# codeMonkey339/Congestion-control-with-BitTorren

Measured on AMD Instinct MI355X. Metric: GiB/s device-resident SHA-1 over 512KB chunks; % of HBM-read roofline, higher is better.
Workload: dtype u32; 1 GPU; 4096 x 524288 B chunks per GPU, device-resident (BASELINE config 2); chunks_per_gpu=4096, chunk_bytes=524288, kernel=split_u4_2prod, kernel_requested=auto, streams=1, parallelism=chunk-sharded x1, no collective

## Files before the change

### congestion-control-with-bittorren_amd/csrc/rt_device.hip

```cpp
#include <algorithm>
#include <atomic>
#include <cctype>
#include <cstdarg>
#include <cstdio>
#include <cstdlib>
#include <cstring>
#include <mutex>
#include <sched.h>
#include <string>
#include <vector>

#include "sha1_runtime_internal.h"

using namespace s1rt;

namespace {
std::atomic<uint64_t> g_launches[kLaunchCounters];

std::string sysfs_line(const char* path) {
    char buf[4096] = {0};
    if (FILE* f = fopen(path, "r")) {
        if (!fgets(buf, sizeof buf, f)) buf[0] = 0;
        fclose(f);
    }
// ... 69 lines not shown
    std::call_once(n.once, [&] {
        if (numa_off()) return;
        cpu_set_t allowed, mine;
        if (!s1host::process_cpus(&allowed)) return;
        constexpr int kMinNearCpus = 4;
        if (device_node_cpus(id, allowed, &mine) < kMinNearCpus || CPU_EQUAL(&mine, &allowed)) return;
        n.set = mine;
        n.ok = true;
    });
    return n.ok ? &n.set : nullptr;
}

const std::vector<cpu_set_t>& receive_domains(int id) {
    struct Dom {
        std::once_flag once;
        std::vector<cpu_set_t> dom;
    };
    static Dom doms[64];
    static const std::vector<cpu_set_t> none;
    if (id < 0 || id >= 64) return none;
    Dom& d = doms[id];
    std::call_once(d.once, [&] {
        cpu_set_t allowed, base;
        if (!s1host::process_cpus(&allowed)) return;
        if (numa_off() || device_node_cpus(id, allowed, &base) == 0) base = allowed;
        s1host::l3_domains(base, &d.dom, [](int cpu) {
            char path[128];
            snprintf(path, sizeof path, "/sys/devices/system/cpu/cpu%d/cache/index3/shared_cpu_list", cpu);
            return sysfs_line(path);
        });
    });
    return d.dom;
}

thread_local int t_dev = 0;

int fail(int code, const char* fmt, ...) {
    char buf[512];
    va_list ap;
    va_start(ap, fmt);
    vsnprintf(buf, sizeof buf, fmt, ap);
    va_end(ap);
    t_err = buf;
    return code;
}

std::string g_probe_err;
Device* g_dev = nullptr;

int device_count() {
    std::call_once(g_once, probe);
    return g_count;
}

int ensure_slots(Device& D, int n) {
    for (int i = 0; i < n && i < kMaxSlots; ++i) {
        Slot& s = D.slot[i];
        if (s.stream) continue;
        HIP_TRY(hipEventCreateWithFlags(&s.done, hipEventDisableTiming));
        HIP_TRY(hipEventCreateWithFlags(&s.copied, hipEventDisableTiming));
        HIP_TRY(hipStreamCreateWithFlags(&s.stream, hipStreamNonBlocking));
    }
    return SHA1CHUNK_OK;
}

int ensure_copy(Device& D) {
    if (!D.copy) HIP_TRY(hipStreamCreateWithFlags(&D.copy, hipStreamNonBlocking));
    return SHA1CHUNK_OK;
}

int get_device(Device** out) {
    if (device_count() <= 0) return fail(SHA1CHUNK_ENODEV, "%s", g_probe_err.c_str());
    if (t_dev < 0 || t_dev >= g_count) return fail(SHA1CHUNK_EINVAL, "bad device %d", t_dev);
    Device& D = g_dev[t_dev];
    HIP_TRY(hipSetDevice(D.id));
    if (!D.ready.load(std::memory_order_acquire)) {
        std::lock_guard<std::mutex> lk(D.mu);
        if (!D.ready.load(std::memory_order_relaxed)) {
            hipDeviceProp_t pr;
            HIP_TRY(hipGetDeviceProperties(&pr, D.id));
            D.cus = pr.multiProcessorCount;
            int rc = ensure_slots(D, 1);
            if (rc) return rc;
            D.ready.store(true, std::memory_order_release);
        }
    }
    *out = &D;
    return SHA1CHUNK_OK;
}

int copies_issued(Slot& s, hipStream_t cs) {
    if (cs == s.stream) return SHA1CHUNK_OK;
    HIP_TRY(hipEventRecord(s.copied, cs));
    HIP_TRY(hipStreamWaitEvent(s.stream, s.copied, 0));
    return SHA1CHUNK_OK;
}

int discard_in_flight(Device& D) {
    for (auto& s : D.slot) {
        if (!s.busy) continue;
        s.busy = false;
        HIP_TRY(hipEventSynchronize(s.done));
    }
    return SHA1CHUNK_OK;
}

int drain_cus_take(Device* D) {
    const int want = static_cast<int>(
        std::max<uint64_t>(1, std::min<uint64_t>({static_cast<uint64_t>(D->cus), 1024, env_u64("SHA1CHUNK_VQ_CUS", 64)})));
    const int budget = static_cast<int>(std::min<uint64_t>(
        static_cast<uint64_t>(D->cus), env_u64("SHA1CHUNK_VQ_CU_BUDGET", static_cast<uint64_t>(D->cus / 2))));
    std::lock_guard<std::mutex> lk(D->drain_mu);
    const int left = budget - D->drain_cus;
    const int take = std::min(want, left);
    if (take < std::min(want, 8)) return 0;
    D->drain_cus += take;
    return take;
}

void drain_cus_give(int dev, int cus) {
    if (dev < 0 || dev >= g_count) return;
    std::lock_guard<std::mutex> lk(g_dev[dev].drain_mu);
    g_dev[dev].drain_cus -= cus;
}

int drain_cus_held() {
    if (!g_dev || t_dev < 0 || t_dev >= g_count) return 0;
    std::lock_guard<std::mutex> lk(g_dev[t_dev].drain_mu);
    return g_dev[t_dev].drain_cus;
}
}

extern "C" {

int s1be_device_count(void) {
    const int n = device_count();
    if (n <= 0) fail(SHA1CHUNK_ENODEV, "%s", g_probe_err.c_str());
    return n;
}

int s1be_set_device(int device) {
    const int n = device_count();
    if (n <= 0) return fail(SHA1CHUNK_ENODEV, "%s", g_probe_err.c_str());
    if (device < 0 || device >= n) return fail(SHA1CHUNK_EINVAL, "device %d of %d", device, n);
    t_dev = device;
    return SHA1CHUNK_OK;
}

const char* s1be_last_error(void) { return t_err.c_str(); }

int s1be_device_pci_bus_id(int device, char* buf, size_t len) {
    const int n = device_count();
    if (n <= 0) return fail(SHA1CHUNK_ENODEV, "%s", g_probe_err.c_str());
    if (device < 0 || device >= n) return fail(SHA1CHUNK_EINVAL, "device %d of %d", device, n);
    if (len > static_cast<size_t>(INT32_MAX)) len = INT32_MAX;
    HIP_TRY(hipDeviceGetPCIBusId(buf, static_cast<int>(len), g_dev[device].id));
    return SHA1CHUNK_OK;
}

int s1be_receive_cpus(int device, unsigned slot, void* mask, size_t len, unsigned* domains) {
    const int n = device_count();
    if (n <= 0) return fail(SHA1CHUNK_ENODEV, "%s", g_probe_err.c_str());
    if (device < 0 || device >= n) return fail(SHA1CHUNK_EINVAL, "device %d of %d", device, n);
    const std::vector<cpu_set_t>& dom = receive_domains(g_dev[device].id);
    if (dom.empty()) return fail(SHA1CHUNK_EINVAL, "no CPU of this process's affinity mask found");
    const cpu_set_t& d = dom[slot % dom.size()];
// ... 18 lines not shown
```

### congestion-control-with-bittorren_amd/csrc/sha1_kernels.h

```cpp
#pragma once

#include <hip/hip_runtime.h>
#include <stdint.h>

struct BatchArgs {
    const uint8_t* base;
    const uint64_t* off;
    const uint32_t* len;
    uint32_t ulen;
    uint32_t n;
    const uint32_t* order;
    uint8_t* dig;
    const uint32_t* init_state;
    uint64_t prefix_bytes;
    uint32_t* out_state;
    const uint32_t* plan;
};

enum LaunchCounter {
    kLaunchLane, kLaunchFused, kLaunchSplit1, kLaunchSplit4, kLaunchSplit11Lane, kLaunchSplit11Shared,
    kLaunchQuad, kLaunchStudy, kLaunchMixed, kLaunchSort, kLaunchDrain, kLaunchCounters
};
void count_launch(LaunchCounter which);

hipError_t launch_lane(const BatchArgs& A, hipStream_t st);
hipError_t launch_fused(const BatchArgs& A, hipStream_t st);
constexpr int kSplitUnitQuad = 416;
bool split_unit_built(int unit_blocks);
hipError_t launch_split(const BatchArgs& A, int unit_blocks, hipStream_t st);
bool split_unit_study_built(int unit_blocks);
hipError_t launch_split_study(const BatchArgs& A, int unit_blocks, hipStream_t st);
uint32_t mixed_grid(uint32_t groups, int cus, uint32_t* hcap);
constexpr uint32_t kBigExact = 4096;
struct BigFix {
    const uint32_t* cnt;
    uint32_t tiles;
    const uint32_t* len;
    const uint32_t* id;
    uint32_t* order;
    uint32_t* sorted_len;
};
hipError_t launch_mixed(const BatchArgs& A, const uint32_t* sorted_len, const BigFix* big, uint32_t* plan, int cus,
                        const int* forced, hipStream_t st);
hipError_t launch_plan_layout(const BatchArgs& A, const uint32_t* sorted_len, const BigFix* big, uint32_t* plan,
                              hipStream_t st);
struct VqDrainArgs {
    const uint8_t* data;
    const uint64_t* off;
    const uint32_t* len;
    const uint8_t* exp;
    const uint32_t* grp;
    const uint32_t* pub;
    const uint32_t* stop;
    uint8_t* alive;
    uint8_t* res;
    uint32_t* done;
    uint32_t* last_done;
    uint8_t* dig;
    uint32_t* claim;
    uint32_t grp_ring;
    uint32_t pad;
    uint64_t idle_ticks;
    uint64_t life_ticks;
};
hipError_t launch_vq_drain(const VqDrainArgs& Q, uint32_t grid, hipStream_t st);

struct PvEntry {
    uint32_t session;
    uint32_t from;
    uint32_t upto;
    uint32_t len;
    uint32_t final;
    uint32_t gen;
    uint32_t pad[2];
};
struct PvArgs {
    const uint8_t* data;
    uint64_t stride;
    const PvEntry* work;
    uint32_t n;
    uint32_t sessions;
    uint32_t* state;
    const uint32_t* expected;
    uint32_t* result;
    uint32_t* done;
    const uint8_t* dummy;
};
hipError_t launch_progress(const PvArgs& P, int depth, hipStream_t st);
hipError_t launch_progress_shared(const PvArgs& P, hipStream_t st);

struct UpdateArgs {
    uint8_t* ctx;
    uint64_t n_contexts;
    const uint32_t* index;
    uint32_t n;
    const uint8_t* base;
    const uint64_t* off;
    const uint32_t* len;
    uint64_t* mid_off;
    uint32_t* mid_len;
    uint32_t* state;
    uint8_t* dig;
};
hipError_t launch_update_init(const UpdateArgs& U, hipStream_t st);
hipError_t launch_update_pre(const UpdateArgs& U, hipStream_t st);
hipError_t launch_update_post(const UpdateArgs& U, hipStream_t st);
hipError_t launch_update_final(const UpdateArgs& U, hipStream_t st);

struct GatherArgs {
    const uint8_t* base;
    const uint64_t* seg_off;
    const uint32_t* seg_len;
// ... 42 lines not shown
```

### congestion-control-with-bittorren_amd/csrc/sha1_kernels.hip

```cpp
#include <hip/hip_runtime.h>
#include <stdint.h>

#include <algorithm>
#include <cstdlib>
#include <cstring>

#include "sha1_fused.hpp"
#include "sha1_split.hpp"

#define PLAN_SPLIT4 0.743
#define PLAN_SPLIT8 0.860
#define PLAN_FUSED4T 1.254
#define PLAN_FUSED4S 1.334
#define PLAN_FUSED8T 2.502
#define PLAN_FUSED8S 2.628
#define PLAN_FUSED_SHARE 0.955

__global__ __launch_bounds__(256) void sha1_lane_kernel(BatchArgs A) {
    const uint32_t e = blockIdx.x * blockDim.x + threadIdx.x;
    if (e >= A.n) return;
    const Entry en = fetch_entry(A, e);
    uint32_t h[5];
    load_init(A, en.id, h);
    lane_blocks(A, en, 0, h);
// ... 790 lines not shown
        for (uint32_t w = 1; w < kMaxCand / 64; ++w) key = min(key, red[w]);
        uint32_t bi = (uint32_t)key;
        if (cmk[2] <= cmk[bi] * 1.005f) bi = 2;
        plan[0] = cmode[bi];
        plan[1] = cmode[bi] == 1 ? 0u : chead[bi];
        plan[2] = cmode[bi] == 1 ? 0u : cf[bi];
#pragma unroll
        for (int i = 1; i < 6; ++i) plan[7 + i] = static_cast<uint32_t>(ts[i] - ts[0]);
#pragma unroll
        for (int i = 1; i < 6; ++i) plan[13 + i] = static_cast<uint32_t>(cs[i] - cs[0]);
#pragma unroll
        for (int i = 0; i < 3; ++i) plan[20 + i] = static_cast<uint32_t>(sub[i] - cs[0]);
        plan[23] = nrun;
#pragma unroll
        for (int i = 0; i < 3; ++i) plan[24 + i] = static_cast<uint32_t>(bsub[i] - cs[0]);
        plan[27] = simcyc;
    }
}

__device__ __forceinline__ uint64_t splitmix64(uint64_t x) {
    uint64_t z = x + 0x9E3779B97F4A7C15ull;
    z = (z ^ (z >> 30)) * 0xBF58476D1CE4E5B9ull;
    z = (z ^ (z >> 27)) * 0x94D049BB133111EBull;
    return z ^ (z >> 31);
}

__global__ __launch_bounds__(kSynthThreads) void synth_fill_kernel(uint8_t* dst, const uint64_t* off,
                                                         const uint32_t* lens, uint32_t ulen,
                                                         uint64_t first, uint64_t seed) {
    const uint64_t c = blockIdx.x;
    const uint32_t len = lens ? lens[c] : ulen;
    uint8_t* out = dst + (off ? off[c] : c * (uint64_t)ulen);
    const uint64_t key = seed ^ ((first + c) << 24);
    const uint32_t nw = len >> 3;
    uint64_t* o = reinterpret_cast<uint64_t*>(out);
    for (uint32_t w = threadIdx.x; w < nw; w += blockDim.x) o[w] = splitmix64(key ^ (uint64_t)w);
    const uint32_t rem = len & 7u;
    if (rem && threadIdx.x == 0) {
        const uint64_t v = splitmix64(key ^ (uint64_t)nw);
        for (uint32_t b = 0; b < rem; ++b) out[8ull * nw + b] = (uint8_t)(v >> (8 * b));
    }
}

__global__ __launch_bounds__(256) void compare_kernel(const uint8_t* dig, const uint8_t* exp,
                                                      uint32_t n, uint8_t* mismatch) {
    const uint32_t i = blockIdx.x * blockDim.x + threadIdx.x;
    if (i >= n) return;
    uint32_t diff = 0;
#pragma unroll
    for (int b = 0; b < 20; ++b) diff |= (uint32_t)(dig[20ull * i + b] ^ exp[20ull * i + b]);
    mismatch[i] = diff ? 1 : 0;
}

hipError_t launch_lane(const BatchArgs& A, hipStream_t st) {
    if (A.n == 0) return hipSuccess;
    const uint32_t grid = (A.n + 255u) / 256u;
    count_launch(kLaunchLane);
    hipLaunchKernelGGL(sha1_lane_kernel, dim3(grid), dim3(256), 0, st, A);
    return hipGetLastError();
}

hipError_t launch_fused(const BatchArgs& A, hipStream_t st) {
    if (A.n == 0) return hipSuccess;
    count_launch(kLaunchFused);
    hipLaunchKernelGGL(sha1_fused_kernel, dim3((A.n + 255u) / 256u), dim3(256), 0, st, A);
    return hipGetLastError();
}

__attribute__((weak)) bool split_unit_study_built(int) { return false; }
__attribute__((weak)) hipError_t launch_split_study(const BatchArgs&, int, hipStream_t) {
    return hipErrorInvalidValue;
}

bool split_unit_built(int u) {
    return u == 1 || u == 4 || u == 11 || u == kSplitUnitQuad || split_unit_study_built(u);
}

static_assert(kSplitThreads<1, kSplitV<1>, 1> == 128, "unit 1: consumer + producer");
static_assert(kSplitThreads<1, kSplitV<4>, kSplitNProd<4>> == 256, "unit 4: consumer, two producers, wave 2 empty");
static_assert(kSplitThreads<2, kSplit8V, 2> == 512 && kSplitThreads<2, kSplit8V & ~kVCoop, 2> == 512,
              "unit 11: the 8-wave layout");
static_assert(kSplitThreads<1, kSplitQuadV, 2> == 256, "unit 416: as unit 4");

hipError_t launch_split(const BatchArgs& A, int unit_blocks, hipStream_t st) {
    if (A.n == 0) return hipSuccess;
    const uint32_t groups = (A.n + 63u) / 64u;
    switch (unit_blocks) {
    case 1:
        count_launch(kLaunchSplit1);
        launch_shape<1, 1>(A, groups, st);
        break;
    case 4:
        count_launch(kLaunchSplit4);
        launch_shape<4, 1, kSplitV<4>, kSplitNProd<4>>(A, groups, st);
        break;
    case 11:
        if (A.off == nullptr && A.order == nullptr) {
            count_launch(kLaunchSplit11Lane);
            launch_shape<2, 2, kSplit8V & ~kVCoop, 2>(A, (groups + 1) / 2, st);
        } else {
            count_launch(kLaunchSplit11Shared);
            launch_shape<2, 2, kSplit8V, 2>(A, (groups + 1) / 2, st);
        }
        break;
    case kSplitUnitQuad:
        count_launch(kLaunchQuad);
        launch_shape<4, 1, kSplitQuadV, 2>(A, (A.n + 15u) / 16u, st);
        break;
    default: return launch_split_study(A, unit_blocks, st);
    }
    return hipGetLastError();
}

uint32_t mixed_grid(uint32_t groups, int cus, uint32_t* hcap) {
    *hcap = std::min<uint32_t>(std::min<uint32_t>(groups, 4u * (uint32_t)cus), kPlanMaxH);
    return groups;
}

hipError_t launch_plan_layout(const BatchArgs& A, const uint32_t* sorted_len, const BigFix* big, uint32_t* plan,
                              hipStream_t st) {
    if (A.n == 0) return hipSuccess;
    const uint32_t groups = (A.n + 63u) / 64u;
    const uint32_t words = (groups + 31u) / 32u;
    uint64_t* lay_tb = reinterpret_cast<uint64_t*>(plan + 64);
    uint32_t* lay_bits = reinterpret_cast<uint32_t*>(lay_tb + words);
    uint32_t* lay_blk = lay_bits + words;
    hipLaunchKernelGGL(plan_layout_kernel, dim3(words), dim3(kLayoutThreads), 0, st, A, sorted_len,
                       big ? *big : BigFix{}, lay_tb, lay_bits, lay_blk);
    return hipGetLastError();
}

hipError_t launch_mixed(const BatchArgs& A, const uint32_t* sorted_len, const BigFix* big, uint32_t* plan, int cus,
                        const int* forced, hipStream_t st) {
    if (A.n == 0) return hipSuccess;
    const uint32_t groups = (A.n + 63u) / 64u;
    uint32_t hcap;
    const uint32_t grid = mixed_grid(groups, cus, &hcap);
    const uint32_t words = (groups + 31u) / 32u;
    uint64_t* lay_tb = reinterpret_cast<uint64_t*>(plan + 64);
    uint32_t* lay_bits = reinterpret_cast<uint32_t*>(lay_tb + words);
    const uint32_t* lay_blk = lay_bits + words;
    count_launch(kLaunchMixed);
    if (!forced) {
        const hipError_t le = launch_plan_layout(A, sorted_len, big, plan, st);
        if (le != hipSuccess) return le;
    }
    hipLaunchKernelGGL(plan_mixed_kernel, dim3(1), dim3(kPlanThreads), 0, st, A, sorted_len,
                       (uint32_t)cus, hcap, forced ? 1 : 0, forced ? (uint32_t)forced[0] : 0u,
                       forced ? (uint32_t)forced[1] : 0u, forced ? (uint32_t)forced[2] : 0u, plan, lay_tb,
                       lay_bits, lay_blk);
    hipError_t e = hipGetLastError();
    if (e != hipSuccess) return e;
    BatchArgs B = A;
    B.plan = plan;
    const char* disp = getenv("SHA1CHUNK_MIXED_DISPATCH");
    const bool persistent = !(disp && !strcmp(disp, "hw"));
    if (persistent)
        hipLaunchKernelGGL(sha1_mixed_persistent_kernel, dim3((uint32_t)cus), dim3(kMixedThreads), 0, st, B,
                           plan + 3);
    else
        hipLaunchKernelGGL(sha1_mixed_kernel, dim3(grid), dim3(kMixedThreads), 0, st, B);
    return hipGetLastError();
}

hipError_t launch_vq_drain(const VqDrainArgs& Q, uint32_t grid, hipStream_t st) {
    count_launch(kLaunchDrain);
    hipLaunchKernelGGL(sha1_vq_drain_kernel, dim3(grid), dim3(kMixedThreads), 0, st, Q);
    return hipGetLastError();
}

hipError_t launch_synth(uint8_t* dst, const uint64_t* off, const uint32_t* lens, uint32_t ulen,
                        uint64_t first, uint64_t count, uint64_t seed, hipStream_t st) {
    if (count == 0) return hipSuccess;
    if (count > kSynthMaxChunks) return hipErrorInvalidValue;
    hipLaunchKernelGGL(synth_fill_kernel, dim3((uint32_t)count), dim3(kSynthThreads), 0, st, dst, off, lens,
                       ulen, first, seed);
    return hipGetLastError();
}

hipError_t launch_compare(const uint8_t* dig, const uint8_t* exp, uint32_t n, uint8_t* mismatch,
                          hipStream_t st) {
    if (n == 0) return hipSuccess;
    hipLaunchKernelGGL(compare_kernel, dim3((n + 255u) / 256u), dim3(256), 0, st, dig, exp, n,
                       mismatch);
    return hipGetLastError();
}

#ifdef SHA1CHUNK_CHECKED
extern "C" __attribute__((visibility("default"))) long long s1be_checked_violations(int reset) {
    int cur = 0, nd = 0;
    if (hipGetDevice(&cur) != hipSuccess || hipGetDeviceCount(&nd) != hipSuccess) return -1;
    long long total = 0;
    for (int d = 0; d < nd; ++d) {
        unsigned int v = 0;
// ... 14 lines not shown
```

### congestion-control-with-bittorren_amd/csrc/sha1_runtime.hip

```cpp
#include <algorithm>
#include <cstdio>
#include <cstdlib>
#include <cstring>
#include <mutex>
#include <numeric>
#include <string>
#include <thread>
#include <vector>

#include "sha1_runtime_internal.h"

using namespace s1rt;

namespace {
int split_unit(size_t n, int cus) {
    if (const char* e = getenv("SHA1CHUNK_SPLIT_UNIT")) return atoi(e);
    if ((n + 15) / 16 <= size_t(std::max(0, cus - drain_cus_held()))) return kSplitUnitQuad;
    const size_t groups = (n + 63) / 64;
    if (groups <= size_t(cus)) return 4;
    if (groups <= size_t(cus) * 2) return 11;
    return 1;
}

hipError_t launch(int kernel, const BatchArgs& A, int cus, hipStream_t st) {
// ... 256 lines not shown
    cut[0] = 0;
    uint64_t acc = 0;
    int d = 1;
    for (size_t i = 0; i < n && d < nd; ++i) {
        acc += lengths[i];
        while (d < nd && acc >= total * (uint64_t)d / (uint64_t)nd) cut[d++] = i + 1;
    }
    std::vector<int> rcs(nd, 0);
    std::vector<std::string> errs(nd);
    std::vector<std::thread> th;
    for (int g = 0; g < nd; ++g) {
        th.emplace_back([&, g] {
            t_dev = g;
            const size_t a = cut[g], b = cut[g + 1];
            if (b > a) {
                std::vector<uint64_t> off(offsets + a, offsets + b);
                rcs[g] = hash_host(base, off.data(), lengths + a, b - a, digests + 20 * a);
                if (rcs[g]) errs[g] = s1be_last_error();
            }
        });
    }
    for (auto& t : th) t.join();
    for (int g = 0; g < nd; ++g)
        if (rcs[g]) return fail(rcs[g], "device %d: %s", g, errs[g].c_str());
    return SHA1CHUNK_OK;
}

}

extern "C" {

int s1be_hash_device_async(const void* d_base, const uint64_t* d_offsets,
                                const uint32_t* d_lengths, size_t n, uint8_t* d_digests,
                                void* stream, int kernel) {
    if (n > 0xffffffffu) return fail(SHA1CHUNK_EINVAL, "n too large");
    if (n && (!d_base || !d_offsets || !d_lengths || !d_digests))
        return fail(SHA1CHUNK_EINVAL, "null device pointer");
    Device* D;
    int rc = get_device(&D);
    if (rc) return rc;
    BatchArgs A{};
    A.base = static_cast<const uint8_t*>(d_base);
    A.off = d_offsets;
    A.len = d_lengths;
    A.n = static_cast<uint32_t>(n);
    A.dig = d_digests;
    hipStream_t st = static_cast<hipStream_t>(stream);
    if ((rc = check_batch(A))) return rc;
    void* scratch = nullptr;
    if (kernel == SHA1CHUNK_KERNEL_AUTO && n > 64) {
        const uint32_t* sorted_len = nullptr;
        uint32_t* plan = nullptr;
        BigFix big{};
        const bool mixed = use_mixed(n, D->cus);
        hipError_t e = sort_by_length_desc(d_lengths, A.n, &A.order, &sorted_len, &plan, &scratch,
                                           mixed ? &big : nullptr, st);
        if (e != hipSuccess) return fail(SHA1CHUNK_EHIP, "length sort: %s", hipGetErrorString(e));
        if (mixed) {
            rc = launch_mixed_checked(A, sorted_len, &big, plan, D->cus, st);
            (void)hipFreeAsync(scratch, st);
            return rc;
        }
    }
    rc = launch_checked(choose_kernel(kernel, n, D->cus), A, st, D->cus);
    if (scratch) (void)hipFreeAsync(scratch, st);
    return rc;
}

int s1be_hash_uniform_async(const void* d_base, uint32_t chunk_len, size_t n,
                                 uint8_t* d_digests, void* stream, int kernel) {
    if (n > 0xffffffffu) return fail(SHA1CHUNK_EINVAL, "n too large");
    if (n && (!d_base || !d_digests)) return fail(SHA1CHUNK_EINVAL, "null device pointer");
    Device* D;
    int rc = get_device(&D);
    if (rc) return rc;
    BatchArgs A{};
    A.base = static_cast<const uint8_t*>(d_base);
    A.ulen = chunk_len;
    A.n = static_cast<uint32_t>(n);
    A.dig = d_digests;
    return launch_checked(choose_kernel(kernel, n, D->cus), A, static_cast<hipStream_t>(stream), D->cus);
}

int s1be_sort_order_async(const uint32_t* d_lengths, size_t n, uint32_t* d_order, uint32_t* d_sorted_len,
                          void* stream) {
    if (n > 0xffffffffu) return fail(SHA1CHUNK_EINVAL, "n too large");
    if (n == 0) return SHA1CHUNK_OK;
    if (!d_lengths || !d_order || !d_sorted_len) return fail(SHA1CHUNK_EINVAL, "null device pointer");
    Device* D;
    if (int rc = get_device(&D)) return rc;
    hipStream_t st = static_cast<hipStream_t>(stream);
    const uint32_t *order = nullptr, *sorted_len = nullptr;
    uint32_t* plan = nullptr;
    void* scratch = nullptr;
    hipError_t e = sort_by_length_desc(d_lengths, static_cast<uint32_t>(n), &order, &sorted_len, &plan, &scratch,
                                       nullptr, st);
    if (e != hipSuccess) return fail(SHA1CHUNK_EHIP, "length sort: %s", hipGetErrorString(e));
    (void)sorted_len;
    e = hipMemcpyAsync(d_order, order, n * sizeof(uint32_t), hipMemcpyDeviceToDevice, st);
    if (e == hipSuccess) e = gather_sorted_lengths(d_lengths, order, d_sorted_len, static_cast<uint32_t>(n), st);
    (void)hipFreeAsync(scratch, st);
    if (e != hipSuccess) return fail(SHA1CHUNK_EHIP, "sort copy: %s", hipGetErrorString(e));
    return SHA1CHUNK_OK;
}

int s1be_mixed_order_async(const uint32_t* d_lengths, const uint64_t* d_offsets, size_t n, uint32_t* d_order,
                           uint32_t* d_sorted_len, void* stream) {
    if (n > 0xffffffffu) return fail(SHA1CHUNK_EINVAL, "n too large");
    if (n == 0) return SHA1CHUNK_OK;
    if (!d_lengths || !d_offsets || !d_order || !d_sorted_len) return fail(SHA1CHUNK_EINVAL, "null device pointer");
    Device* D;
    if (int rc = get_device(&D)) return rc;
    hipStream_t st = static_cast<hipStream_t>(stream);
    BatchArgs A{};
    A.base = reinterpret_cast<const uint8_t*>(d_offsets);
    A.off = d_offsets;
    A.len = d_lengths;
    A.n = static_cast<uint32_t>(n);
    const uint32_t* sorted_len = nullptr;
    uint32_t* plan = nullptr;
    void* scratch = nullptr;
    BigFix big{};
    hipError_t e = sort_by_length_desc(d_lengths, A.n, &A.order, &sorted_len, &plan, &scratch, &big, st);
    if (e != hipSuccess) return fail(SHA1CHUNK_EHIP, "length sort: %s", hipGetErrorString(e));
    e = launch_plan_layout(A, sorted_len, &big, plan, st);
    if (e == hipSuccess) e = hipMemcpyAsync(d_order, A.order, n * sizeof(uint32_t), hipMemcpyDeviceToDevice, st);
    if (e == hipSuccess) e = gather_sorted_lengths(d_lengths, A.order, d_sorted_len, A.n, st);
    (void)hipFreeAsync(scratch, st);
    if (e != hipSuccess) return fail(SHA1CHUNK_EHIP, "mixed order: %s", hipGetErrorString(e));
    return SHA1CHUNK_OK;
}

int s1be_compare_device_async(const uint8_t* d_digests, const uint8_t* d_expected, size_t n,
                                   uint8_t* d_mismatch, void* stream) {
    if (n > 0xffffffffu - 255u) return fail(SHA1CHUNK_EINVAL, "n too large: at most 2^32 - 256 per call");
    if (n && (!d_digests || !d_expected || !d_mismatch))
        return fail(SHA1CHUNK_EINVAL, "null device pointer");
    Device* D;
    int rc = get_device(&D);
    if (rc) return rc;
    hipError_t e = launch_compare(d_digests, d_expected, static_cast<uint32_t>(n), d_mismatch,
                                  static_cast<hipStream_t>(stream));
    if (e != hipSuccess) return fail(SHA1CHUNK_EHIP, "compare launch: %s", hipGetErrorString(e));
    return SHA1CHUNK_OK;
}

int s1be_hash_batch(const void* base, const uint64_t* offsets, const uint32_t* lengths,
                         size_t n, uint8_t* digests, unsigned flags) {
    if (n == 0) return SHA1CHUNK_OK;
    if (!base || !offsets || !lengths || !digests) return fail(SHA1CHUNK_EINVAL, "null pointer");
    if (n > 0xffffffffu) return fail(SHA1CHUNK_EINVAL, "n too large");
    if (flags & SHA1CHUNK_DEVICE) {
        Device* D;
        int rc = get_device(&D);
        if (rc) return rc;
        std::lock_guard<std::mutex> lk(D->mu);
        hipStream_t st = D->slot[0].stream;
        if ((rc = s1be_hash_device_async(base, offsets, lengths, n, digests, st,
                                              SHA1CHUNK_KERNEL_AUTO)))
            return rc;
        HIP_TRY(hipStreamSynchronize(st));
        return SHA1CHUNK_OK;
    }
    const uint8_t* b = static_cast<const uint8_t*>(base);
    if (flags & SHA1CHUNK_ALL_DEVICES) return hash_host_all(b, offsets, lengths, n, digests);
    return hash_host(b, offsets, lengths, n, digests);
// ... 126 lines not shown
```

### congestion-control-with-bittorren_amd/csrc/sha1_split.hpp

```cpp
#ifndef SHA1_SPLIT_HPP
#define SHA1_SPLIT_HPP

#include "sha1_lane.hpp"

constexpr int kWBlockBytes = 20 * 1024;

constexpr int kVWK = 1;
constexpr int kVUnmask = 4;
constexpr int kVRead10 = 8;
constexpr int kVSkipWave2 = 64;
constexpr int kVLayout8 = 128;
constexpr int kVCross = 256;
constexpr int kVProbe = 2048;
constexpr int kVCoop = 8192;
constexpr int kVQuad = 8192 * 4;

template <int U>
constexpr int kSplitV = U == 4 ? (kVWK | kVUnmask | kVSkipWave2 | kVRead10 | kVCoop)
                               : U == 3 ? kVUnmask : (kVWK | kVUnmask);
template <int U>
constexpr int kSplitNProd = U == 4 ? 2 : 1;
constexpr int kSplit8V = kVWK | kVUnmask | kVLayout8 | kVCross | kVCoop;
constexpr int kSplitQuadV = kVWK | kVUnmask | kVSkipWave2 | kVCoop | kVQuad;
template <int PAIRS, int V, int NPROD>
constexpr int kSplitThreads = (V & kVLayout8) ? 512 : 64 * PAIRS * (1 + NPROD) + ((V & kVSkipWave2) ? 64 : 0);


__device__ __forceinline__ void split_barrier() {
    __builtin_amdgcn_s_waitcnt(0xC07F);
    asm volatile("s_barrier" ::: "memory");
}

__device__ __forceinline__ void split_barrier_timed(uint64_t& acc) {
    __builtin_amdgcn_s_waitcnt(0xC07F);
    const uint64_t t0 = __builtin_amdgcn_s_memtime();
    asm volatile("s_barrier" ::: "memory");
    acc += __builtin_amdgcn_s_memtime() - t0;
}

template <int T, bool WK>
struct SchedWrite {
    __device__ __forceinline__ static void run(uint32_t (&w)[16], uint8_t* slot, int lane) {
        if constexpr (T < 80) {
            if constexpr (T >= 16) sched_step<T>(w);
            if constexpr ((T & 3) == 3) {
                constexpr int j = (T - 3) & 15;
                constexpr uint32_t k = WK ? round_k<T>() : 0u;
                *reinterpret_cast<uint4*>(slot + (T >> 2) * 1024 + lane * 16) =
                    make_uint4(w[j] + k, w[j + 1] + k, w[j + 2] + k, w[j + 3] + k);
            }
            SchedWrite<T + 1, WK>::run(w, slot, lane);
        }
    }
};

__device__ __forceinline__ uint32_t total_blocks(uint32_t len) {
    return (len >> 6) + (((len & 63u) < 56u) ? 1u : 2u);
}

__device__ __forceinline__ void tail_block_words(const Entry& en, uint32_t k, uint32_t (&w)[16]) {
    const uint32_t nfull = en.len >> 6, rem = en.len & 63u;
    const uint64_t bits = (uint64_t)en.len * 8ull;
    if (k < nfull) {
        load_block16(en.p + 64ull * k, w);
#pragma unroll
        for (int j = 0; j < 16; ++j) w[j] = bswap(w[j]);
    } else if (k == nfull) {
        if (rem) {
            load_block_partial(en.p + 64ull * k, rem, w);
        } else {
#pragma unroll
            for (int j = 0; j < 16; ++j) w[j] = 0u;
        }
#pragma unroll
        for (int j = 0; j < 16; ++j) w[j] = pad_word(bswap(w[j]), j, (int)rem);
        if (rem < 56u) {
            w[14] = (uint32_t)(bits >> 32);
            w[15] = (uint32_t)bits;
        }
    } else {
#pragma unroll
        for (int j = 0; j < 14; ++j) w[j] = 0u;
        w[14] = (uint32_t)(bits >> 32);
        w[15] = (uint32_t)bits;
    }
}

template <int U, bool WK, int NPROD = 1>
__device__ __forceinline__ void produce_block(uint32_t k, uint32_t (&w)[16], uint8_t* ring, int lane,
                                              uint64_t* bw = nullptr) {
    const uint32_t m = k / U, j = k - m * U;
    SchedWrite<0, WK>::run(w, ring + ((m & 1u) * U + j) * kWBlockBytes, lane);
    if (NPROD == 1 ? j == U - 1 : (U == NPROD || (k & 1u) == 1u)) {
        if (bw)
            split_barrier_timed(*bw);
        else
            split_barrier();
    }
// ... 219 lines not shown
struct QuadSchedWrite {
    __device__ __forceinline__ static void run(uint32_t (&w)[16], uint8_t* slot, bool j1, bool j2,
                                               const uint32_t (&kq)[5]) {
        if constexpr (T < 80) {
            if constexpr (T >= 16) sched_step<T>(w);
            if constexpr ((T & 15) == 15) {
                constexpr int q = T >> 4;
                uint32_t o[4];
#pragma unroll
                for (int i = 0; i < 4; ++i) {
                    const uint32_t lo = j1 ? w[4 + i] : w[i], hi = j1 ? w[12 + i] : w[8 + i];
                    o[i] = (j2 ? hi : lo) + kq[q];
                }
                *reinterpret_cast<uint4*>(slot + q * 1024) = make_uint4(o[0], o[1], o[2], o[3]);
            }
            QuadSchedWrite<T + 1>::run(w, slot, j1, j2, kq);
        }
    }
};

template <int U>
__device__ __forceinline__ void quad_produce_block(uint32_t k, uint32_t (&w)[16], uint8_t* ring, int lane,
                                                   const uint32_t (&kq)[5]) {
    const uint32_t m = k / U, j = k - m * U;
    QuadSchedWrite<0>::run(w, ring + ((m & 1u) * U + j) * kQuadBlockBytes + lane * 16, (lane & 1) != 0,
                           (lane & 2) != 0, kq);
    if ((k & 1u) == 1u && ((k >> 1) % (U / 2)) + 2 >= U / 2) split_barrier();
}

__device__ __forceinline__ void quad_block_words(const uint32_t (&x)[4], uint32_t (&w)[16]) {
    uint32_t y[4];
#pragma unroll
    for (int i = 0; i < 4; ++i) y[i] = bswap(x[i]);
#pragma unroll
    for (int i = 0; i < 4; ++i) {
        w[i] = quad_bcast<0>(y[i]);
        w[4 + i] = quad_bcast<1>(y[i]);
        w[8 + i] = quad_bcast<2>(y[i]);
        w[12 + i] = quad_bcast<3>(y[i]);
    }
}

__device__ __forceinline__ void quad_load_stage(const u32x4u* src, uint32_t s, uint32_t (&x)[8]) {
#pragma unroll
    for (int b = 0; b < 2; ++b) unpack4(x + 4 * b, src[8u * s + 4u * b]);
}

template <int U>
__device__ __forceinline__ void quad_produce_stage(const u32x4u* src, uint32_t s, uint32_t S, uint32_t (&cur)[8],
                                                   uint8_t* ring, int lane, const uint32_t (&kq)[5]) {
    uint32_t x0[4] = {cur[0], cur[1], cur[2], cur[3]}, x1[4] = {cur[4], cur[5], cur[6], cur[7]};
    if (s + 4 < S) quad_load_stage(src, s + 4, cur);
    uint32_t w[16];
    quad_block_words(x0, w);
    quad_produce_block<U>(2 * s, w, ring, lane, kq);
    quad_block_words(x1, w);
    quad_produce_block<U>(2 * s + 1, w, ring, lane, kq);
}

template <int U, int V>
__device__ __forceinline__ void quad_consume_all(const BatchArgs& A, const Entry& en, bool valid, uint32_t T,
                                                 uint32_t units, const uint8_t* ring, int lane, uint32_t wg) {
    uint32_t h[5];
    load_init(A, en.id, h);
    uint32_t Wa[20], Wb[20];
    split_barrier();
    quad_read_w(ring + lane * 16, Wa);
    __builtin_amdgcn_s_waitcnt(0x0070);
    const uint32_t Tmin = __builtin_amdgcn_readfirstlane(wave_min(valid ? T : 0xffffffffu));
    const uint32_t full = min(Tmin, units * U) / (2 * U) * (2 * U);
    uint32_t k = 0;
    uint64_t bw = 0;
    const uint64_t t0 = (V & kVProbe) ? __builtin_amdgcn_s_memtime() : 0;
    for (; k < full; k += 2 * U) QuadConsumeUnits<U, 0, V, false>::run(k, T, h, Wa, Wb, ring, lane, bw);
    for (; k < units * U; k += 2 * U) QuadConsumeUnits<U, 0, V, true>::run(k, T, h, Wa, Wb, ring, lane, bw);
    if constexpr ((V & kVProbe) != 0) {
        const uint64_t tot = __builtin_amdgcn_s_memtime() - t0;
        if (lane == 0) probe_store(A, wg * 16u, bw, tot, units * U);
        return;
    }
    if (valid && (lane & 3) == 0) emit(A, en.id, h);
}

template <int U, int V, int NPROD>
__device__ __forceinline__ void quad_split_body(const BatchArgs& A, uint8_t* ring, uint32_t wg) {
    static_assert((U == 4 || U == 8) && NPROD == 2 && (V & kVSkipWave2) != 0 && (V & kVWK) != 0 &&
                      (V & kVUnmask) != 0,
                  "quad shape: 4- or 8-block units, two producers on waves 1 and 3, W+K shipped");
    int wave = __builtin_amdgcn_readfirstlane(threadIdx.x >> 6);
    if (wave == 2) return;
    const bool producer = wave != 0;
    const uint32_t pidx = wave == 3 ? 1u : 0u;
    const int lane = threadIdx.x & 63;
    bool valid;
    const Entry en = lane_entry(A, wg * 16u + ((uint32_t)lane >> 2), min(wg * 16u, A.n - 1u), valid);
    const uint32_t T = valid ? (A.out_state ? (en.len >> 6) : total_blocks(en.len)) : 0u;
    const uint32_t Tmax = __builtin_amdgcn_readfirstlane(wave_max(T));
    const uint32_t units = (Tmax + 2 * U - 1) / (2 * U) * 2;
    if (!producer) {
        quad_consume_all<U, V>(A, en, valid, T, units, ring, lane, wg);
        return;
    }
    uint32_t kq[5];
#pragma unroll
    for (int q = 0; q < 5; ++q) {
        const uint32_t t = 16u * q + 4u * ((uint32_t)lane & 3u);
        kq[q] = t < 20 ? K0 : t < 40 ? K1 : t < 60 ? K2 : K3;
    }
    const uint32_t S = bulk_stages(en, valid);
    const u32x4u* src = reinterpret_cast<const u32x4u*>(en.p) + (lane & 3);
    uint32_t C0[8], C1[8];
    uint32_t s = pidx;
    if (s < S) quad_load_stage(src, s, C0);
    if (s + 2 < S) quad_load_stage(src, s + 2, C1);
    for (; s + 2 < S; s += 4) {
        quad_produce_stage<U>(src, s, S, C0, ring, lane, kq);
        quad_produce_stage<U>(src, s + 2, S, C1, ring, lane, kq);
    }
    if (s < S) {
        quad_produce_stage<U>(src, s, S, C0, ring, lane, kq);
        s += 2;
    }
    for (; 2 * s < units * U; s += 2) {
#pragma unroll
        for (int half = 0; half < 2; ++half) {
            const uint32_t k = 2 * s + half;
            uint32_t w[16];
            if (k < T) tail_block_words(en, k, w);
            quad_produce_block<U>(k, w, ring, lane, kq);
        }
    }
    split_barrier();
}

template <int U, int PAIRS, int V, int NPROD>
__device__ __forceinline__ void split_body(const BatchArgs& A, uint8_t* lds, uint32_t wg) {
    if constexpr ((V & kVQuad) != 0) {
        static_assert(PAIRS == 1, "quad shape: one consumer per workgroup");
        quad_split_body<U, V, NPROD>(A, lds, wg);
        return;
    }
    constexpr bool WK = (V & kVWK) != 0;
    static_assert((V & kVQuad) != 0 || PAIRS * 2 * U * kWBlockBytes <= 160 * 1024, "LDS");
    static_assert((V & kVQuad) != 0 || NPROD == 1 || (PAIRS == 1 && (U == 2 * NPROD || U == NPROD)) ||
                      (PAIRS == 2 && U == NPROD && (V & kVLayout8) != 0),
                  "two producers: one stage (U = 4) or one block (U = 2, 8-wave layout) each per unit");
    int wave = __builtin_amdgcn_readfirstlane(threadIdx.x >> 6);
    if constexpr ((V & kVSkipWave2) != 0) {
        static_assert(NPROD == 2 && PAIRS == 1, "skip-wave layout is for two producers");
        if (wave == 2) return;
        if (wave > 2) wave -= 1;
    }
    int pair = wave % PAIRS;
    bool producer = wave >= PAIRS;
    uint32_t pidx = producer ? (uint32_t)(wave - PAIRS) / PAIRS : 0u;
    if constexpr ((V & kVLayout8) != 0) {
        static_assert(PAIRS == 2 && NPROD == 2, "8-wave layout: two pairs, two producers each");
        if (wave == 4 || wave == 6) return;
        producer = (wave & 1) != 0;
        pair = producer ? (((wave >> 1) & 1) ^ ((V & kVCross) ? 1 : 0)) : (wave >> 1);
        pidx = producer ? (uint32_t)(wave >> 2) : 0u;
    }
    const int lane = threadIdx.x & 63;
    uint8_t* ring = lds + pair * (2 * U * kWBlockBytes);
    const uint32_t group = wg * PAIRS + (uint32_t)pair;
    bool valid;
    const Entry en = lane_entry(A, group * 64u + (uint32_t)lane, fallback_entry(A, group), valid);
    const uint32_t T = valid ? (A.out_state ? (en.len >> 6) : total_blocks(en.len)) : 0u;
    uint32_t Tmax = __builtin_amdgcn_readfirstlane(wave_max(T));
    if constexpr (PAIRS > 1) {
        uint32_t* slots = reinterpret_cast<uint32_t*>(lds);
        if (!producer && lane == 0) slots[pair] = Tmax;
        __syncthreads();
#pragma unroll
        for (int q = 0; q < PAIRS; ++q) Tmax = max(Tmax, slots[q]);
        Tmax = __builtin_amdgcn_readfirstlane(Tmax);
        __syncthreads();
    }
    const uint32_t units = (Tmax + 2 * U - 1) / (2 * U) * 2;

    if (producer) {
        const uint32_t S = bulk_stages(en, valid);
        if constexpr (U == NPROD) {
// ... 104 lines not shown
```

Measured before the change: 344.1 GiB/s.

## Place quad consumer wave on a claimed SIMD via per-CU atomic table

Adds a per-CU global claim table so each workgroup of the quad split kernel atomically claims SIMD 0 or 2 and reassigns wave roles, putting the consumer wave and the skipped wave on chosen SIMDs and the producers on the others. The aim is to keep consumers from co-resident workgroups off the same SIMD and so spread compute evenly. It costs a global atomic spin per workgroup, two extra barriers, a release atomic at exit, and relies on the HW_ID/XCC_ID register layout. A diagnostic kernel and an env knob to force or disable the placement are also added.

```diff
diff --git a/congestion-control-with-bittorren_amd/csrc/quad_claim.hpp b/congestion-control-with-bittorren_amd/csrc/quad_claim.hpp
--- /dev/null
+++ b/congestion-control-with-bittorren_amd/csrc/quad_claim.hpp
@@ -0,0 +1,73 @@
+#ifndef QUAD_CLAIM_HPP
+#define QUAD_CLAIM_HPP
+
+#include <stdint.h>
+
+#if defined(__HIPCC__) || defined(__CUDACC__)
+#define QUAD_CLAIM_FN __host__ __device__ inline
+#else
+#define QUAD_CLAIM_FN inline
+#endif
+
+constexpr uint32_t kQuadClaimWords = 4096;
+constexpr uint32_t kQuadClaimSimd0 = 1u;
+constexpr uint32_t kQuadClaimSimd2 = 2u;
+
+constexpr uint32_t kQuadSimdAuto = 0;
+constexpr uint32_t kQuadSimdOff = 1;
+constexpr uint32_t kQuadSimdForce0 = 2;
+constexpr uint32_t kQuadSimdForce2 = 3;
+
+constexpr uint32_t kQuadNoSimd = 0xffffffffu;
+
+QUAD_CLAIM_FN uint32_t quad_cu_index(uint32_t xcc_id, uint32_t hw_id) {
+    const uint32_t xcc = xcc_id & 15u, se = (hw_id >> 13) & 7u, sh = (hw_id >> 12) & 1u, cu = (hw_id >> 8) & 15u;
+    return ((xcc * 8u + se) * 2u + sh) * 16u + cu;
+}
+QUAD_CLAIM_FN uint32_t quad_simd_id(uint32_t hw_id) { return (hw_id >> 4) & 3u; }
+
+struct QuadClaim {
+    uint32_t next = kQuadClaimSimd0;
+    uint32_t held = 0;
+};
+QUAD_CLAIM_FN void quad_claim_step(QuadClaim& c, uint32_t before) {
+    if ((before & c.next) == 0) {
+        c.held = c.next;
+        c.next = 0;
+    } else {
+        c.next = c.next == kQuadClaimSimd0 ? kQuadClaimSimd2 : 0u;
+    }
+}
+QUAD_CLAIM_FN uint32_t quad_release_mask(uint32_t held) { return ~held; }
+
+QUAD_CLAIM_FN uint32_t quad_consumer_simd(uint32_t mode, uint32_t held) {
+    if (mode == kQuadSimdForce0) return 0u;
+    if (mode == kQuadSimdForce2) return 2u;
+    if (mode == kQuadSimdOff) return kQuadNoSimd;
+    return held == kQuadClaimSimd0 ? 0u : held == kQuadClaimSimd2 ? 2u : kQuadNoSimd;
+}
+
+QUAD_CLAIM_FN void quad_roles(const uint32_t (&simd)[4], uint32_t cs, uint32_t (&role)[4]) {
+    if (cs != 0u && cs != 2u) {
+        for (int w = 0; w < 4; ++w) role[w] = (uint32_t)w;
+        return;
+    }
+    int wc = -1, wl = -1;
+    for (int w = 0; w < 4; ++w)
+        if (wc < 0 && simd[w] == cs) wc = w;
+    if (wc < 0) wc = 0;
+    for (int w = 0; w < 4; ++w)
+        if (wl < 0 && w != wc && simd[w] == (cs ^ 2u)) wl = w;
+    if (wl < 0) wl = wc == 3 ? 2 : 3;
+    uint32_t producers = 0;
+    for (int w = 0; w < 4; ++w) {
+        if (w == wc)
+            role[w] = 0u;
+        else if (w == wl)
+            role[w] = 2u;
+        else
+            role[w] = producers++ == 0 ? 1u : 3u;
+    }
+}
+
+#endif
diff --git a/congestion-control-with-bittorren_amd/csrc/rt_device.hip b/congestion-control-with-bittorren_amd/csrc/rt_device.hip
--- a/congestion-control-with-bittorren_amd/csrc/rt_device.hip
+++ b/congestion-control-with-bittorren_amd/csrc/rt_device.hip
@@ -175,6 +175,7 @@
             D.cus = pr.multiProcessorCount;
             int rc = ensure_slots(D, 1);
             if (rc) return rc;
+            HIP_TRY(quad_claim_reset());
             D.ready.store(true, std::memory_order_release);
         }
     }
diff --git a/congestion-control-with-bittorren_amd/csrc/sha1_kernels.h b/congestion-control-with-bittorren_amd/csrc/sha1_kernels.h
--- a/congestion-control-with-bittorren_amd/csrc/sha1_kernels.h
+++ b/congestion-control-with-bittorren_amd/csrc/sha1_kernels.h
@@ -14,8 +14,12 @@
     const uint32_t* init_state;
     uint64_t prefix_bytes;
     uint32_t* out_state;
-    const uint32_t* plan;
+    union {
+        const uint32_t* plan;
+        uint64_t quad_simd;
+    };
 };
+static_assert(sizeof(BatchArgs) == 80, "kernel argument layout");
 
 enum LaunchCounter {
     kLaunchLane, kLaunchFused, kLaunchSplit1, kLaunchSplit4, kLaunchSplit11Lane, kLaunchSplit11Shared,
@@ -28,6 +32,8 @@
 constexpr int kSplitUnitQuad = 416;
 bool split_unit_built(int unit_blocks);
 hipError_t launch_split(const BatchArgs& A, int unit_blocks, hipStream_t st);
+hipError_t launch_quad_diag(const BatchArgs& A, uint32_t* rows, hipStream_t st);
+hipError_t quad_claim_reset();
 bool split_unit_study_built(int unit_blocks);
 hipError_t launch_split_study(const BatchArgs& A, int unit_blocks, hipStream_t st);
 uint32_t mixed_grid(uint32_t groups, int cus, uint32_t* hcap);
diff --git a/congestion-control-with-bittorren_amd/csrc/sha1_kernels.hip b/congestion-control-with-bittorren_amd/csrc/sha1_kernels.hip
--- a/congestion-control-with-bittorren_amd/csrc/sha1_kernels.hip
+++ b/congestion-control-with-bittorren_amd/csrc/sha1_kernels.hip
@@ -896,6 +896,15 @@
               "unit 11: the 8-wave layout");
 static_assert(kSplitThreads<1, kSplitQuadV, 2> == 256, "unit 416: as unit 4");
 
+static int quad_simd_mode() {
+    const char* e = getenv("SHA1CHUNK_QUAD_SIMD");
+    if (!e || !strcmp(e, "auto")) return (int)kQuadSimdAuto;
+    if (!strcmp(e, "off")) return (int)kQuadSimdOff;
+    if (!strcmp(e, "0")) return (int)kQuadSimdForce0;
+    if (!strcmp(e, "2")) return (int)kQuadSimdForce2;
+    return -1;
+}
+
 hipError_t launch_split(const BatchArgs& A, int unit_blocks, hipStream_t st) {
     if (A.n == 0) return hipSuccess;
     const uint32_t groups = (A.n + 63u) / 64u;
@@ -917,13 +926,42 @@
             launch_shape<2, 2, kSplit8V, 2>(A, (groups + 1) / 2, st);
         }
         break;
-    case kSplitUnitQuad:
+    case kSplitUnitQuad: {
+        const int mode = quad_simd_mode();
+        if (mode < 0) return hipErrorInvalidValue;
+        BatchArgs Q = A;
+        Q.quad_simd = (uint64_t)mode;
         count_launch(kLaunchQuad);
-        launch_shape<4, 1, kSplitQuadV, 2>(A, (A.n + 15u) / 16u, st);
+        launch_shape<4, 1, kSplitQuadV, 2>(Q, (A.n + 15u) / 16u, st);
         break;
+    }
     default: return launch_split_study(A, unit_blocks, st);
     }
     return hipGetLastError();
+}
+
+__global__ __launch_bounds__((kSplitThreads<1, kSplitQuadV, 2>)) void sha1_quad_diag_kernel(BatchArgs A,
+                                                                                          QuadDiag* rows) {
+    __shared__ __attribute__((aligned(16))) uint8_t lds[kSplitLdsBytes<4, 1, kSplitQuadV>];
+    quad_split_body<4, kSplitQuadV | kVDiag, 2>(A, lds, blockIdx.x, rows);
+}
+
+hipError_t launch_quad_diag(const BatchArgs& A, uint32_t* rows, hipStream_t st) {
+    if (A.n == 0) return hipSuccess;
+    const int mode = quad_simd_mode();
+    if (mode < 0) return hipErrorInvalidValue;
+    BatchArgs Q = A;
+    Q.quad_simd = (uint64_t)mode;
+    count_launch(kLaunchQuad);
+    hipLaunchKernelGGL(sha1_quad_diag_kernel, dim3((A.n + 15u) / 16u), dim3(kSplitThreads<1, kSplitQuadV, 2>), 0, st,
+                       Q, reinterpret_cast<QuadDiag*>(rows));
+    return hipGetLastError();
+}
+
+hipError_t quad_claim_reset() {
+    void* table = nullptr;
+    const hipError_t e = hipGetSymbolAddress(&table, HIP_SYMBOL(g_quad_claim));
+    return e != hipSuccess ? e : hipMemset(table, 0, sizeof(uint32_t) * kQuadClaimWords);
 }
 
 uint32_t mixed_grid(uint32_t groups, int cus, uint32_t* hcap) {
diff --git a/congestion-control-with-bittorren_amd/csrc/sha1_runtime.hip b/congestion-control-with-bittorren_amd/csrc/sha1_runtime.hip
--- a/congestion-control-with-bittorren_amd/csrc/sha1_runtime.hip
+++ b/congestion-control-with-bittorren_amd/csrc/sha1_runtime.hip
@@ -362,6 +362,28 @@
     return launch_checked(choose_kernel(kernel, n, D->cus), A, static_cast<hipStream_t>(stream), D->cus);
 }
 
+int s1be_quad_diag_async(const void* d_base, const uint64_t* d_offsets, const uint32_t* d_lengths,
+                         uint32_t chunk_len, size_t n, uint8_t* d_digests, uint32_t* d_rows, void* stream) {
+    if (n > 0xffffffffu) return fail(SHA1CHUNK_EINVAL, "n too large");
+    if (n && (!d_base || !d_digests || !d_rows || !d_offsets != !d_lengths))
+        return fail(SHA1CHUNK_EINVAL, "null device pointer");
+    if (reinterpret_cast<uintptr_t>(d_rows) & 7u) return fail(SHA1CHUNK_EALIGN, "rows must be 8-byte aligned");
+    Device* D;
+    int rc = get_device(&D);
+    if (rc) return rc;
+    BatchArgs A{};
+    A.base = static_cast<const uint8_t*>(d_base);
+    A.off = d_offsets;
+    A.len = d_lengths;
+    A.ulen = chunk_len;
+    A.n = static_cast<uint32_t>(n);
+    A.dig = d_digests;
+    if ((rc = check_batch(A))) return rc;
+    const hipError_t e = launch_quad_diag(A, d_rows, static_cast<hipStream_t>(stream));
+    if (e != hipSuccess) return fail(SHA1CHUNK_EHIP, "kernel launch: %s", hipGetErrorString(e));
+    return SHA1CHUNK_OK;
+}
+
 int s1be_sort_order_async(const uint32_t* d_lengths, size_t n, uint32_t* d_order, uint32_t* d_sorted_len,
                           void* stream) {
     if (n > 0xffffffffu) return fail(SHA1CHUNK_EINVAL, "n too large");
diff --git a/congestion-control-with-bittorren_amd/csrc/sha1_split.hpp b/congestion-control-with-bittorren_amd/csrc/sha1_split.hpp
--- a/congestion-control-with-bittorren_amd/csrc/sha1_split.hpp
+++ b/congestion-control-with-bittorren_amd/csrc/sha1_split.hpp
@@ -1,6 +1,7 @@
 #ifndef SHA1_SPLIT_HPP
 #define SHA1_SPLIT_HPP
 
+#include "quad_claim.hpp"
 #include "sha1_lane.hpp"
 
 constexpr int kWBlockBytes = 20 * 1024;
@@ -14,6 +15,7 @@
 constexpr int kVProbe = 2048;
 constexpr int kVCoop = 8192;
 constexpr int kVQuad = 8192 * 4;
+constexpr int kVDiag = 8192 * 8;
 
 template <int U>
 constexpr int kSplitV = U == 4 ? (kVWK | kVUnmask | kVSkipWave2 | kVRead10 | kVCoop)
@@ -399,23 +401,108 @@
     if (valid && (lane & 3) == 0) emit(A, en.id, h);
 }
 
+static __device__ uint32_t g_quad_claim[kQuadClaimWords];
+
+__device__ __forceinline__ uint32_t quad_hw_id() {
+    return __builtin_amdgcn_s_getreg((31u << 11) | (0u << 6) | 4u);
+}
+__device__ __forceinline__ uint32_t quad_this_cu(uint32_t hw) {
+    return quad_cu_index(__builtin_amdgcn_s_getreg((3u << 11) | (0u << 6) | 20u), hw);
+}
+
+constexpr uint32_t kQuadDiagWords = 16;
+struct QuadDiag {
+    uint32_t cu, simd, held, mode;
+    uint64_t t_entry;
+    uint64_t t_claimed;
+    uint64_t t_exit;
+    uint64_t t_released;
+    uint32_t wave, written, pad[2];
+};
+static_assert(sizeof(QuadDiag) == 4 * kQuadDiagWords, "placement row");
+
 template <int U, int V, int NPROD>
-__device__ __forceinline__ void quad_split_body(const BatchArgs& A, uint8_t* ring, uint32_t wg) {
+__device__ __forceinline__ void quad_split_body(const BatchArgs& A, uint8_t* ring, uint32_t wg,
+                                                QuadDiag* diag = nullptr) {
     static_assert((U == 4 || U == 8) && NPROD == 2 && (V & kVSkipWave2) != 0 && (V & kVWK) != 0 &&
                       (V & kVUnmask) != 0,
                   "quad shape: 4- or 8-block units, two producers on waves 1 and 3, W+K shipped");
+    constexpr bool kDiag = (V & kVDiag) != 0;
+    __shared__ __attribute__((aligned(16))) uint32_t placed[kDiag ? 8 : 4];
     int wave = __builtin_amdgcn_readfirstlane(threadIdx.x >> 6);
+    const int lane = threadIdx.x & 63;
+    const uint32_t mode = (uint32_t)A.quad_simd;
+    const uint32_t hw = quad_hw_id();
+    bool valid;
+    const Entry en = lane_entry(A, wg * 16u + ((uint32_t)lane >> 2), min(wg * 16u, A.n - 1u), valid);
+    uint32_t mine = quad_simd_id(hw);
+    if (mode != kQuadSimdOff && wave == 0) {
+        if constexpr (kDiag) {
+            const uint64_t t = __builtin_amdgcn_s_memrealtime();
+            asm volatile("" ::: "memory");
+            if (lane == 0) placed[4] = (uint32_t)t, placed[5] = (uint32_t)(t >> 32);
+        }
+        QuadClaim c;
+        if (mode == kQuadSimdAuto && lane == 0) {
+            uint32_t* word = &g_quad_claim[quad_this_cu(hw)];
+            while (c.next)
+                quad_claim_step(c, __hip_atomic_fetch_or(word, c.next, __ATOMIC_RELAXED, __HIP_MEMORY_SCOPE_AGENT));
+        }
+        mine |= c.held << 8;
+    }
+    const uint32_t T = valid ? (A.out_state ? (en.len >> 6) : total_blocks(en.len)) : 0u;
+    const uint32_t Tmax = __builtin_amdgcn_readfirstlane(wave_max(T));
+    const uint32_t units = (Tmax + 2 * U - 1) / (2 * U) * 2;
+    uint32_t held = 0;
+    if (mode != kQuadSimdOff) {
+        if (lane == 0) placed[wave] = mine;
+        split_barrier();
+        const uint4 p = *reinterpret_cast<const uint4*>(placed);
+        const uint32_t p0 = __builtin_amdgcn_readfirstlane(p.x);
+        const uint32_t simd[4] = {p0 & 3u, __builtin_amdgcn_readfirstlane(p.y) & 3u,
+                                  __builtin_amdgcn_readfirstlane(p.z) & 3u,
+                                  __builtin_amdgcn_readfirstlane(p.w) & 3u};
+        held = p0 >> 8;
+        uint32_t role[4];
+        quad_roles(simd, quad_consumer_simd(mode, held), role);
+        split_barrier();
+        wave = (int)(wave == 0 ? role[0] : wave == 1 ? role[1] : wave == 2 ? role[2] : role[3]);
+    }
     if (wave == 2) return;
     const bool producer = wave != 0;
     const uint32_t pidx = wave == 3 ? 1u : 0u;
-    const int lane = threadIdx.x & 63;
-    bool valid;
-    const Entry en = lane_entry(A, wg * 16u + ((uint32_t)lane >> 2), min(wg * 16u, A.n - 1u), valid);
-    const uint32_t T = valid ? (A.out_state ? (en.len >> 6) : total_blocks(en.len)) : 0u;
-    const uint32_t Tmax = __builtin_amdgcn_readfirstlane(wave_max(T));
-    const uint32_t units = (Tmax + 2 * U - 1) / (2 * U) * 2;
     if (!producer) {
+        uint64_t t_entry = 0, t_claimed = 0;
+        if constexpr (kDiag) {
+            t_claimed = __builtin_amdgcn_s_memrealtime();
+            if (mode != kQuadSimdOff)
+                t_entry = ((uint64_t)(uint32_t)__builtin_amdgcn_readfirstlane(placed[5]) << 32) |
+                          (uint32_t)__builtin_amdgcn_readfirstlane(placed[4]);
+            else
+                t_entry = t_claimed;
+        }
         quad_consume_all<U, V>(A, en, valid, T, units, ring, lane, wg);
+        if constexpr (kDiag) {
+            __builtin_amdgcn_s_waitcnt(0);
+            QuadDiag row = {quad_this_cu(hw), quad_simd_id(hw), held, mode, t_entry, t_claimed, 0, 0,
+                            threadIdx.x >> 6, 1u, {0u, 0u}};
+            asm volatile("" ::: "memory");
+            row.t_exit = __builtin_amdgcn_s_memrealtime();
+            asm volatile("" ::: "memory");
+            if (lane == 0) {
+                uint32_t was = 0;
+                if (held)
+                    was = __hip_atomic_fetch_and(&g_quad_claim[quad_this_cu(hw)], quad_release_mask(held),
+                                                 __ATOMIC_RELAXED, __HIP_MEMORY_SCOPE_AGENT);
+                asm volatile("s_waitcnt vmcnt(0)" ::"v"(was) : "memory");
+                row.t_released = __builtin_amdgcn_s_memrealtime();
+                diag[wg] = row;
+            }
+            return;
+        }
+        if (held && lane == 0)
+            __hip_atomic_fetch_and(&g_quad_claim[quad_this_cu(hw)], quad_release_mask(held), __ATOMIC_RELAXED,
+                                   __HIP_MEMORY_SCOPE_AGENT);
         return;
     }
     uint32_t kq[5];
```

Result: no change. 344.7 GiB/s, median of 6 (+0.2%).
